# oarodriguez/PhD-QMCLib

Measured on AMD Instinct MI355X. Metric: walker-steps/sec, higher is better.
Workload: dtype f64

## Files before the change

### phd_qmclib_amd/csrc/qmc_kernels.h

```cpp
#pragma once

#include "qmc_device.h"
#include "qmc_sorted64.h"
#include "qmc_sorted128.h"

static constexpr int BLOCK = 256;

static constexpr int BLOCK64 = 64;
template <int G>
struct WalkBlock {
    static constexpr int N = (G == 64) ? BLOCK64 : BLOCK;
};

template <int GPB>
__device__ __forceinline__ long long walker_of_block(unsigned b, int grp)
{
    if (GPB == 1)
        return ((long long)(b >> 7) << 7) + ((b & 7u) << 4) + ((b & 127u) >> 3);
    return (long long)b * GPB + grp;
}

template <int G, int P, bool PAD, bool ZC, bool DMC = false>
struct StepLds {
    static constexpr int NROWS =
        DMC ? SortedCot<false, true, false>::ROWS : 5;
    static constexpr int SORTED =
        (G == 64 && P == 2 && !ZC)   ? NROWS * SortedRows<128>::ROW
        : (G == 64 && P == 1 && !ZC) ? NROWS * SortedRows<64>::ROW
                                     : 0;
    static constexpr int GENERAL = GroupLds<G, P, ZC>::DOUBLES;
    static constexpr int DOUBLES = SORTED > GENERAL ? SORTED : GENERAL;
};

__device__ __forceinline__ long long qmc_uniform(long long v)
{
    const int lo = __builtin_amdgcn_readfirstlane((int)v);
    const int hi = __builtin_amdgcn_readfirstlane((int)(v >> 32));
    return ((long long)hi << 32) | (unsigned int)lo;
}
__device__ __forceinline__ int qmc_opaque(int v)
{
    asm volatile("" : "+v"(v));
    return v;
}
__device__ __forceinline__ double qmc_uniform_f64(double v)
{
    return __longlong_as_double(qmc_uniform(__double_as_longlong(v)));
}
__device__ __forceinline__ double qmc_lane_f64(double v, int k)
{
    const long long b = __double_as_longlong(v);
    const int lo = __builtin_amdgcn_readlane((int)b, k);
    const int hi = __builtin_amdgcn_readlane((int)(b >> 32), k);
    return __longlong_as_double(((long long)hi << 32) | (unsigned int)lo);
}

template <int P>
__device__ __forceinline__ void vmc_accept_lanes(const int (&lab)[P], int n,
                                                 int &src0, int &src1)
{
    src0 = 0;
    src1 = 0;
#pragma unroll
    for (int p = 0; p < P; ++p) {
        const unsigned long long b0 = __ballot(lab[p] == 0);
        const unsigned long long b1 = __ballot(lab[p] == 1);
        if (b0) src0 = ((int)__ffsll((long long)b0) - 1) | (p << 6);
        if (b1) src1 = ((int)__ffsll((long long)b1) - 1) | (p << 6);
    }
    if (n == 1) src1 = src0;
}
template <int P>
__device__ __forceinline__ unsigned int vmc_read_slot(const uint32_t (&wd)[P],
                                                      int src)
{
    unsigned int r = 0u;
#pragma unroll
    for (int p = 0; p < P; ++p)
        if ((src >> 6) == p)
            r = (unsigned)__builtin_amdgcn_readlane((int)wd[p], src & 63);
    return r;
}

static constexpr int LB_P1 = 7;
static constexpr int LB_DMC_P2 = 5;
static constexpr int LB_VMC_P2 = 4;
constexpr int lb_waves(int G, int P, bool ZC, int p2)
{
    return (G == 64 && P == 1) ? LB_P1 : (G == 64 && P == 2 && !ZC) ? p2 : 1;
}


template <int P>
struct DmcSpare {
    static constexpr bool ON = P == 1;
};

static constexpr int RESORT_EVERY = 4;

struct EvalArgs {
    const double *pos;
    double *wf, *energy;
    double *ith, *drift;
    long long nconf;
};

template <int G, int P, bool PAD, bool ZC, typename R = double>
__global__ void __launch_bounds__(WalkBlock<G>::N, lb_waves(G, P, ZC, 1))
evaluate_kernel(const DevModel *__restrict__ mp, EvalArgs a)
{
    const DevModel &m = *mp;
    [[maybe_unused]] constexpr int QMC_SEC_OFF = 0;
    QMC_SECTION("top");
    extern __shared__ double smem[];
    constexpr int GPB = WalkBlock<G>::N / G;
    const int grp = threadIdx.x / G, gl = threadIdx.x % G;
    double *lds = smem + (size_t)grp * GroupLds<G, P, ZC>::DOUBLES;
    const long long w = walker_of_block<GPB>(blockIdx.x, grp);
    const bool active = w < a.nconf;
    if (GPB == 1 && !active) return;
    const long long wr = active ? w : 0;
    const int n = walker_n<G, P, PAD>(m);
    double z[P], z1[P], F[P], ei[P], E, wf;
#pragma unroll
    for (int p = 0; p < P; ++p) {
        int i = lane_particle<G, P, PAD>(m, gl, p);
        z1[p] = (i < n) ? a.pos[wr * n + i] : 0.0;
        z[p] = wrap_box(z1[p], m.L);
    }
    eval_walker<G, P, PAD, true, true, ZC, R>(m, z, z1, gl, lds, F, ei, E, wf);
    if (!active) return;
#pragma unroll
    for (int p = 0; p < P; ++p) {
        int i = lane_particle<G, P, PAD>(m, gl, p);
        if (i < n) {
            if (a.ith) a.ith[w * n + i] = ei[p];
            if (a.drift) a.drift[w * n + i] = F[p];
        }
    }
    if (gl == 0) {
        if (a.wf) a.wf[w] = wf;
        if (a.energy) a.energy[w] = E;
    }
}

struct PrepArgs {
    const double *pos;
    double *drift, *energy;
    long long nconf;
};

template <int G, int P, bool PAD, bool ZC, typename R = double>
__global__ void __launch_bounds__(WalkBlock<G>::N, lb_waves(G, P, ZC, 1))
prepare_kernel(const DevModel *__restrict__ mp, PrepArgs a)
{
    const DevModel &m = *mp;
    [[maybe_unused]] constexpr int QMC_SEC_OFF = 0;
    QMC_SECTION("top");
    extern __shared__ double smem[];
    constexpr int GPB = WalkBlock<G>::N / G;
    const int grp = threadIdx.x / G, gl = threadIdx.x % G;
    double *lds = smem + (size_t)grp * GroupLds<G, P, ZC>::DOUBLES;
    const long long w = walker_of_block<GPB>(blockIdx.x, grp);
    const bool active = w < a.nconf;
    if (GPB == 1 && !active) return;
    const long long wr = active ? w : 0;
    const int n = walker_n<G, P, PAD>(m);
    double z[P], z1[P], F[P], ei[P], E, wf;
#pragma unroll
    for (int p = 0; p < P; ++p) {
        int i = lane_particle<G, P, PAD>(m, gl, p);
        z1[p] = (i < n) ? a.pos[wr * n + i] : 0.0;
        z[p] = wrap_box(z1[p], m.L);
    }
    eval_walker<G, P, PAD, false, false, ZC, R>(m, z, z1, gl, lds, F, ei, E,
                                                wf);
    if (!active) return;
#pragma unroll
    for (int p = 0; p < P; ++p) {
        int i = lane_particle<G, P, PAD>(m, gl, p);
        if (i < n) a.drift[w * n + i] = F[p];
    }
    if (gl == 0) a.energy[w] = E;
}

struct alignas(64) VmcRec {
    double wf;
    double ecarry;
    double sum_e, sum_e2;
    long long n_acc;
    long long spare[3];
};
static_assert(sizeof(VmcRec) == 64, "one record = 8 eight-byte words");
typedef unsigned int VmcRecWords __attribute__((ext_vector_type(16)));
#define QMC_CONST __attribute__((address_space(4)))
__device__ __forceinline__ double vmc_rec_word(const VmcRecWords &r, int k)
{
    return __hiloint2double((int)r[2 * k + 1], (int)r[2 * k]);
}

struct VmcArgs {
    double *pos;
    unsigned short *label;
    VmcRec *rec;
    double *ser_wf, *ser_e;
    unsigned char *ser_stat;
    double *ser_pos;
    const double *tape;
    long long tape_steps;
    long long tape_idx;
    long long W;
    long long y;
    unsigned int nsteps;
    int forced;
    int reset_sums;
    int gaussian;
    unsigned int step;
    unsigned int chain0;
    unsigned long long seed;
    double move_spread;
};

template <int G, int P, bool ZC>
struct VmcFused {
    static constexpr bool ON = G == 64 && !ZC && (P == 1 || P == 2);
};

template <int G, int P, bool PAD, bool ZC, bool LEAN, typename R = double,
          bool STEADY = false>
__global__ void __launch_bounds__(WalkBlock<G>::N, lb_waves(G, P, ZC, LB_VMC_P2))
vmc_step_kernel(const DevModel *__restrict__ mp, VmcArgs a)
{
    static_assert(LEAN || !STEADY, "the steady variant is a LEAN kernel");
    const DevModel &m = *mp;
    [[maybe_unused]] constexpr int QMC_SEC_OFF = 0;
    QMC_SECTION("top");
    extern __shared__ double smem[];
    constexpr int GPB = WalkBlock<G>::N / G;
    const int grp = threadIdx.x / G, gl = threadIdx.x % G;
    static_assert(StepLds<G, P, PAD, ZC>::DOUBLES >= GroupLds<G, P, ZC>::DOUBLES,
                  "eval_walker is the fallback on the same LDS region");
    double *lds = smem + (size_t)grp * StepLds<G, P, PAD, ZC>::DOUBLES;
    const long long w = walker_of_block<GPB>(blockIdx.x, grp);
    const bool active = w < a.W;
    if (GPB == 1 && !active) return;
    const long long wr = active ? w : 0;
    const int n = walker_n<G, P, PAD>(m);
    const unsigned int slot = a.chain0 + (unsigned int)wr;
    const bool forced = !STEADY && a.forced != 0;
    const bool reset_sums = !STEADY && a.reset_sums != 0;

    const long long wl = (G == 64) ? qmc_uniform(wr) : wr;
    double wf_cur, e_cur, se = 0.0, se2 = 0.0;
    long long na = 0;
    if constexpr (G == 64) {
        const VmcRecWords r = *(const QMC_CONST VmcRecWords *)(a.rec + wl);
        wf_cur = vmc_rec_word(r, 0);
        e_cur = vmc_rec_word(r, 1);
        se = vmc_rec_word(r, 2);
        se2 = vmc_rec_word(r, 3);
        na = __double_as_longlong(vmc_rec_word(r, 4));
        if (reset_sums) { se = 0.0; se2 = 0.0; na = 0; }
    } else {
        wf_cur = a.rec[wl].wf;
        e_cur = a.rec[wl].ecarry;
    }

    constexpr bool FUSED = STEADY && VmcFused<G, P, ZC>::ON;
    double zc[P];
    int labc[P];
    int src0 = 0, src1 = 0;
    if constexpr (FUSED) {
#pragma unroll
        for (int p = 0; p < P; ++p) {
            int i = lane_particle<G, P, PAD>(m, gl, p);
            zc[p] = (i < n) ? a.pos[wr * n + i] : 0.0;
            labc[p] = (i < n) ? (int)a.label[wr * n + i] : i;
        }
        vmc_accept_lanes<P>(labc, n, src0, src1);
    }
    bool any_acc = false;
    const unsigned int nst = FUSED ? a.nsteps : 1u;
    bool acc = false;
    [[maybe_unused]] const int gl_top = gl;
    for (unsigned int s = 0; s < nst; ++s) {
    const unsigned int step = a.step + s;
    const int gl = FUSED ? qmc_opaque(gl_top) : gl_top;
    QMC_SECTION("load+philox+wrap");
    double zn[P];
    int labn[P];
    double ua = 1.0;
    unsigned int aw0 = 0u, aw1 = 0u;
    bool has0 = false, has1 = false;
    bool outside = false;
    [[maybe_unused]] uint32_t wacc[P];
#pragma unroll
    for (int p = 0; p < P; ++p) {
        wacc[p] = 0u;
        int i = lane_particle<G, P, PAD>(m, gl, p);
        double zp;
        if constexpr (FUSED) {
            zp = zc[p];
            labn[p] = labc[p];
        } else {
            zp = (i < n) ? a.pos[wr * n + i] : 0.0;
            labn[p] = (i < n) ? (int)a.label[wr * n + i] : i;
        }
        const unsigned li = (unsigned)labn[p];
        double d = 0.0;
        if (!forced && i < n) {
            if (!LEAN && a.tape) {
                double tv = a.tape[(wr * a.tape_steps + a.tape_idx) * (n + 1) + li];
                d = a.gaussian ? a.move_spread * tv
                               : (tv - 0.5) * a.move_spread;
            } else if (!LEAN && a.gaussian) {
                double g0, g1;
                philox_normal2(a.seed, slot, step, li, STREAM_VMC_MOVE, g0,
                               g1);
                d = a.move_spread * g0;
            } else {
                uint32_t w0, w1;
                vmc_move_block(a.seed, slot, step, li, w0, w1);
                d = vmc_move_unit(w0) * a.move_spread;
                if constexpr (FUSED) {
                    wacc[p] = w1;
                } else {
                    if (li == 0u) { aw0 = w1; has0 = true; }
                    if (li == 1u || n == 1) { aw1 = w1; has1 = true; }
                }
            }
        }
        zn[p] = wrap_box(zp + d, m.L);
        if (forced) outside = outside || zn[p] != zp;
    }
    if constexpr (FUSED) {
        aw0 = vmc_read_slot<P>(wacc, src0);
        aw1 = vmc_read_slot<P>(wacc, src1);
    }
    QMC_SECTION("resort");
    constexpr bool S64 = G == 64 && P == 1 && !ZC;
    constexpr bool S128 = G == 64 && P == 2 && !ZC;
    bool fast = false;
    if (forced)
        outside = __builtin_amdgcn_ballot_w64(outside) != 0ull;
    if constexpr (S64) {
        fast = !m.is_ideal && !outside &&
               sort_lanes64(zn[0], labn[0], gl, PAD ? n : 64) &&
               (PAD ? far_partner_ok_ring(m, zn[0], gl, n)
                    : far_partner_ok64(m, zn[0], gl));
    } else if constexpr (S128) {
        fast = !m.is_ideal && !outside && (!PAD || (n & 1) == 0) &&
               sort_rows128(zn, labn, gl, PAD ? n / 2 : 64) &&
               (PAD ? far_partner_ok_ring128(m, zn, gl, n / 2)
                    : far_partner_ok128(m, zn, gl));
    }
    if constexpr (S64 || S128) {
        if (!fast && !m.is_ideal && gl == 0 && active)
            atomicAdd(m.diag, 1ull);
    } else if constexpr (G == 64 && P == 1) {
        if (!forced) {
            anchor_seam(zn[0], labn[0], n);
            if ((a.step % RESORT_EVERY) == 0)
                resort_linear<G>(zn[0], labn[0], gl,
                                 a.step / RESORT_EVERY, n);
        }
    } else if constexpr (SlotMap<G, P>::CONSECUTIVE) {
        if (!forced) {
            anchor_seam_rows<P>(zn, labn, n);
            if ((a.step % RESORT_EVERY) == 0)
                resort_linear_rows<P>(zn, labn, gl, a.step / RESORT_EVERY, n);
        }
    } else if (!forced && (a.step % RESORT_EVERY) == 0)
        resort_step<G, P>(zn, labn, gl, a.step / RESORT_EVERY, n, m.L,
                          m.half_L, lanes_in_use<G, PAD>(m));
    constexpr bool TWO_PASS = G == 64;
    double F[P], ei[P], e_new = 0.0, wf_new;
    if (S64 && fast) {
        if constexpr (S64)
            eval_sorted64<R, true, false, false, PAD>(
                m, zn[0], gl, lds, F[0], e_new, wf_new);
    } else if (S128 && fast) {
        if constexpr (S128)
            eval_sorted128<R, true, false, false, PAD>(m, zn, gl, lds, F,
                                                       e_new, wf_new);
    } else {
        double z1[P];
#pragma unroll
        for (int p = 0; p < P; ++p) {
            int i = lane_particle<G, P, PAD>(m, gl, p);
            z1[p] = (outside && i < n) ? a.pos[wr * n + i] : zn[p];
        }
        if constexpr (TWO_PASS)
            eval_walker<G, P, PAD, true, false, ZC, R, false, false>(
                m, zn, z1, gl, lds, F, ei, e_new, wf_new);
        else
            eval_walker<G, P, PAD, true, false, ZC, R>(m, zn, z1, gl, lds, F,
                                                       ei, e_new, wf_new);
    }
    QMC_SECTION("metropolis+store");
    if (FUSED) {
        ua = u53(aw0, aw1);
    } else if (!forced) {
        if (!LEAN && a.tape) {
            ua = a.tape[(wr * a.tape_steps + a.tape_idx) * (n + 1) + n];
        } else if (!LEAN && a.gaussian) {
            double u1;
            philox_uniform2(a.seed, slot, step, 0u, STREAM_VMC_ACCEPT, ua,
                            u1);
        } else {
            const unsigned long long bal0 = __ballot(has0);
            const unsigned long long bal1 = __ballot(has1);
            unsigned int hi, lo;
            if (G == 64) {
                const int src0 = __builtin_amdgcn_readfirstlane(
                    (int)__ffsll((long long)bal0) - 1) & 63;
                const int src1 = __builtin_amdgcn_readfirstlane(
                    (int)__ffsll((long long)bal1) - 1) & 63;
                hi = (unsigned)__builtin_amdgcn_readlane((int)aw0, src0);
                lo = (unsigned)__builtin_amdgcn_readlane((int)aw1, src1);
            } else {
                const int base = (threadIdx.x & 63) - gl;
                const unsigned long long gmask = (1ull << (G & 63)) - 1ull;
                const int src0 = base + ((__ffsll((long long)((bal0 >> base) &
                                                              gmask)) - 1) & (G - 1));
                const int src1 = base + ((__ffsll((long long)((bal1 >> base) &
                                                              gmask)) - 1) & (G - 1));
                hi = (unsigned)__shfl((int)aw0, src0, 64);
                lo = (unsigned)__shfl((int)aw1, src1, 64);
            }
            ua = u53(hi, lo);
        }
    }
    if (!active) return;
    if constexpr (FUSED) {
        const double w0 = qmc_uniform_f64(wf_new);
        acc = ua <= 0.0 || w0 > wf_cur;
        if (!acc) acc = w0 > 0.5 * log_pos(ua) + wf_cur;
        acc = __builtin_amdgcn_readfirstlane((int)acc) != 0;
    } else {
        acc = forced || ua <= 0.0 || wf_new > wf_cur;
        if (!acc) acc = wf_new > 0.5 * log_pos(ua) + wf_cur;
        if (G == 64) acc = __builtin_amdgcn_readfirstlane((int)acc) != 0;
    }
    if (acc) {
        if constexpr (TWO_PASS) {
            QMC_SECTION("energy_pass");
            QMC_SECTION_PHASE(QMC_NSEC / 2);
            double wf_unused;
            if (S64 && fast) {
                if constexpr (S64)
                    eval_sorted64<R, false, true, true, PAD>(
                        m, zn[0], gl, lds, F[0], e_new, wf_unused);
            } else if (S128 && fast) {
                if constexpr (S128)
                    eval_sorted128<R, false, true, true, PAD>(
                        m, zn, gl, lds, F, e_new, wf_unused);
            } else {
                double z1[P];
#pragma unroll
                for (int p = 0; p < P; ++p) {
                    int i = lane_particle<G, P, PAD>(m, gl, p);
                    z1[p] = (outside && i < n) ? a.pos[wr * n + i] : zn[p];
                }
                eval_walker<G, P, PAD, false, false, ZC, R, true, true>(
                    m, zn, z1, gl, lds, F, ei, e_new, wf_unused);
            }
            QMC_SECTION_PHASE(0);
            QMC_SECTION("store");
        }
        if constexpr (FUSED) {
#pragma unroll
            for (int p = 0; p < P; ++p) {
                zc[p] = zn[p];
                labc[p] = labn[p];
            }
            vmc_accept_lanes<P>(labc, n, src0, src1);
            any_acc = true;
        } else {
#pragma unroll
            for (int p = 0; p < P; ++p) {
                int i = lane_particle<G, P, PAD>(m, gl, p);
                if (i < n && !forced) {
                    a.pos[w * n + i] = zn[p];
                    a.label[w * n + i] = (unsigned short)labn[p];
                }
            }
        }
        if (!FUSED) {
            wf_cur = wf_new;
            e_cur = e_new;
        }
    }
    if constexpr (FUSED) {
        if (acc) {
            wf_cur = qmc_uniform_f64(wf_new);
            const double e2 = qmc_lane_f64(e_new, 2);
            const double e3 = qmc_lane_f64(e_new, 3);
            e_cur = qmc_lane_f64(e_new, 1);
            se = se + e2;
            se2 = fma(e3, e3, se2);
            na = na + 1;
        } else {
            se = se + e_cur;
            se2 = fma(e_cur, e_cur, se2);
        }
        se = qmc_uniform_f64(se);
        se2 = qmc_uniform_f64(se2);
        continue;
    }
    if (!LEAN && a.ser_pos) {
#pragma unroll
        for (int p = 0; p < P; ++p) {
            int i = lane_particle<G, P, PAD>(m, gl, p);
            if (i < n) {
                const bool moved = acc && !forced;
                const int lb = moved ? labn[p] : (int)a.label[w * n + i];
                a.ser_pos[(a.y * a.W + w) * n + lb] =
                    moved ? zn[p] : a.pos[w * n + i];
            }
        }
    }
    if (G == 64) {
        const double sum1 = se + e_cur;
        const double sum2 = fma(e_cur, e_cur, se2);
        const long long na1 = qmc_uniform(na + (acc ? 1 : 0));
        double v = __longlong_as_double((gl == 4) ? na1 : 0ll);
        v = (gl == 0) ? wf_cur : v;
        v = (gl == 1) ? e_cur : v;
        v = (gl == 2) ? sum1 : v;
        v = (gl == 3) ? sum2 : v;
        if (gl < 8) reinterpret_cast<double *>(a.rec + wl)[gl] = v;
    }
    if (gl == 0) {
        if (G != 64) {
            VmcRec *r = a.rec + w;
            if (!reset_sums) { se = r->sum_e; se2 = r->sum_e2; na = r->n_acc; }
            r->wf = wf_cur;
            r->ecarry = e_cur;
            r->sum_e = se + e_cur;
            r->sum_e2 = fma(e_cur, e_cur, se2);
            r->n_acc = na + (acc ? 1 : 0);
        }
        if (!LEAN) {
            if (a.ser_wf) a.ser_wf[a.y * a.W + w] = wf_cur;
            if (a.ser_e) a.ser_e[a.y * a.W + w] = e_cur;
            if (a.ser_stat) a.ser_stat[a.y * a.W + w] = acc ? 1 : 0;
        }
    }
    }
    if constexpr (FUSED) {
        QMC_SECTION("fused_store");
        if (any_acc) {
#pragma unroll
            for (int p = 0; p < P; ++p) {
                int i = lane_particle<G, P, PAD>(m, gl, p);
                if (i < n) {
                    a.pos[w * n + i] = zc[p];
                    a.label[w * n + i] = (unsigned short)labc[p];
                }
            }
        }
        double v = __longlong_as_double((gl == 4) ? qmc_uniform(na) : 0ll);
        v = (gl == 0) ? wf_cur : v;
        v = (gl == 1) ? e_cur : v;
        v = (gl == 2) ? se : v;
        v = (gl == 3) ? se2 : v;
        if (gl < 8) reinterpret_cast<double *>(a.rec + wl)[gl] = v;
    }
    QMC_SECTION("end");
}

struct DmcCtl {
    long long prev_nw;
    long long nw;
    double ref_energy;
    double total_energy, total_weight;
    double e_t, w_t;
    long long spare_nw;
    unsigned int step;
    unsigned int pad;
};

struct EvolveArgs {
    const double *ppos, *pdrift, *penergy;
    double *cpos, *cdrift, *cenergy, *cweight;
    const unsigned short *plabel;
    unsigned short *clabel;
    double *eslot;
    const long long *ref;
    const DmcCtl *ctl;
    const double *g_tape;
    double *spare;
    long long maxw;
    double dt, sigma;
    unsigned long long seed;
    unsigned int slot0;
    int fix_stale;
};

template <int G, int P, bool PAD, bool ZC, typename R = double>
__global__ void __launch_bounds__(WalkBlock<G>::N, lb_waves(G, P, ZC, LB_DMC_P2))
dmc_evolve_kernel(const DevModel *__restrict__ mp, EvolveArgs a)
{
    const DevModel &m = *mp;
    [[maybe_unused]] constexpr int QMC_SEC_OFF = 0;
    extern __shared__ double smem[];
    constexpr int GPB = WalkBlock<G>::N / G;
    const int grp = threadIdx.x / G, gl = threadIdx.x % G;
    static_assert(StepLds<G, P, PAD, ZC, true>::DOUBLES >=
                      GroupLds<G, P, ZC>::DOUBLES,
                  "eval_walker is the fallback on the same LDS region");
    double *lds = smem + (size_t)grp * StepLds<G, P, PAD, ZC, true>::DOUBLES;
    const long long s = walker_of_block<GPB>(blockIdx.x, grp);
    const long long nw = a.ctl->nw;
    if ((GPB == 1 ? s : (long long)blockIdx.x * GPB) >= nw) return;
    QMC_SECTION("top");
    const bool active = s < nw;
    const long long sr = active ? s : 0;
    const int n = walker_n<G, P, PAD>(m);
    const unsigned int step = a.ctl->step;
    const double ref_energy = a.ctl->ref_energy;
    const long long spare_nw = a.ctl->spare_nw;
    const long long su = (G == 64) ? qmc_uniform(sr) : sr;
    const long long par = a.ref[su];
    double e_par = 0.0, e_slot = 0.0;
    if (G == 64) {
        e_par = a.penergy[par];
        e_slot = a.eslot[su];
    }

    QMC_SECTION("load+philox+wrap");
    double z[P];
    int lab[P];
#pragma unroll
    for (int p = 0; p < P; ++p) {
        int i = lane_particle<G, P, PAD>(m, gl, p);
        double zz = 0.0;
        lab[p] = i;
        if (i < n) {
            double z0 = a.ppos[par * n + i];
            double f0 = a.pdrift[par * n + i];
            const int li = (int)a.plabel[par * n + i];
            lab[p] = li;
            double g;
            if (a.g_tape) {
                g = a.g_tape[sr * n + li];
            } else if (DmcSpare<P>::ON && (step & 1u) && sr < spare_nw) {
                g = a.spare[sr * n + li];
            } else {
                double g0, g1;
                dmc_normal2(a.seed, a.slot0 + (unsigned)sr, step >> 1,
                            (unsigned)li, g0, g1);
                g = (step & 1u) ? g1 : g0;
                if (DmcSpare<P>::ON && !(step & 1u) && active)
                    a.spare[sr * n + li] = g1;
            }
            double zn = z0 + 2 * f0 * a.dt + a.sigma * g;
            zz = wrap_box(zn, m.L);
        }
        z[p] = zz;
    }
    QMC_SECTION("resort");
    constexpr bool S64 = G == 64 && P == 1 && !ZC;
    constexpr bool S128 = G == 64 && P == 2 && !ZC;
    bool fast = false;
    if constexpr (S64) {
        fast = !m.is_ideal && sort_lanes64(z[0], lab[0], gl, PAD ? n : 64) &&
               (PAD ? far_partner_ok_ring(m, z[0], gl, n)
                    : far_partner_ok64(m, z[0], gl));
    } else if constexpr (S128) {
        fast = !m.is_ideal && (!PAD || (n & 1) == 0) &&
               sort_rows128(z, lab, gl, PAD ? n / 2 : 64) &&
               (PAD ? far_partner_ok_ring128(m, z, gl, n / 2)
                    : far_partner_ok128(m, z, gl));
    }
    if constexpr (S64 || S128) {
        if (!fast && !m.is_ideal && gl == 0 && active)
            atomicAdd(m.diag, 1ull);
    } else if constexpr (G == 64 && P == 1) {
        anchor_seam(z[0], lab[0], n);
        if ((step % RESORT_EVERY) == 0)
            resort_linear<G>(z[0], lab[0], gl, step / RESORT_EVERY, n);
    } else if constexpr (SlotMap<G, P>::CONSECUTIVE) {
        anchor_seam_rows<P>(z, lab, n);
        if ((step % RESORT_EVERY) == 0)
            resort_linear_rows<P>(z, lab, gl, step / RESORT_EVERY, n);
    } else if ((step % RESORT_EVERY) == 0)
        resort_step<G, P>(z, lab, gl, step / RESORT_EVERY, n, m.L,
                          m.half_L, lanes_in_use<G, PAD>(m));
#pragma unroll
    for (int p = 0; p < P; ++p) {
        int i = lane_particle<G, P, PAD>(m, gl, p);
        if (active && i < n) {
            a.cpos[s * n + i] = z[p];
            a.clabel[s * n + i] = (unsigned short)lab[p];
        }
    }
    double F[P], ei[P], e_next, wf;
    if (S64 && fast) {
        if constexpr (S64)
            eval_sorted64<R, false, true, false, PAD>(m, z[0], gl, lds, F[0],
                                                      e_next, wf);
    } else if (S128 && fast) {
        if constexpr (S128)
            eval_sorted128<R, false, true, false, PAD>(m, z, gl, lds, F,
                                                       e_next, wf);
    } else
        eval_walker<G, P, PAD, false, false, ZC, R>(m, z, z, gl, lds, F, ei,
                                                    e_next, wf);
    QMC_SECTION("weight+store");
    if (!active) return;
#pragma unroll
    for (int p = 0; p < P; ++p) {
        int i = lane_particle<G, P, PAD>(m, gl, p);
        if (i < n) a.cdrift[s * n + i] = F[p];
    }
    if (gl == 0) {
        if (G != 64) { e_par = a.penergy[par]; e_slot = a.eslot[s]; }
        double e_old = a.fix_stale ? e_par : e_slot;
        double mean_energy = (e_next + e_old) / 2;
        a.cenergy[s] = e_next;
        a.cweight[s] = -a.dt * (mean_energy - ref_energy);
        a.eslot[s] = e_par;
    }
    QMC_SECTION("end");
}
```

Before: 759.6 million.

## Precompute Metropolis acceptance uniforms in lane-parallel chunks across fused VMC steps

In the fused steady VMC kernel, the per-step acceptance uniform is no longer taken from the label-0/label-1 particles' Philox words, which needed ballots after every accept plus readlane selection. Every 30 steps, lanes 4..63 each generate one Philox block for a future step, pair adjacent lanes via DPP to form the 53-bit uniform, and compute its clamped log once, storing a zero-mask ballot. Each step then reads the precomputed log-uniform with a readlane. This removes per-step ballot and readlane work and the per-step log from the serial path. In exchange it adds a batched Philox and log pass every 30 steps and relies on the precomputed stream matching the original acceptance draws.

```diff
diff --git a/phd_qmclib_amd/csrc/qmc_kernels.h b/phd_qmclib_amd/csrc/qmc_kernels.h
--- a/phd_qmclib_amd/csrc/qmc_kernels.h
+++ b/phd_qmclib_amd/csrc/qmc_kernels.h
@@ -53,33 +53,6 @@
     const int lo = __builtin_amdgcn_readlane((int)b, k);
     const int hi = __builtin_amdgcn_readlane((int)(b >> 32), k);
     return __longlong_as_double(((long long)hi << 32) | (unsigned int)lo);
-}
-
-template <int P>
-__device__ __forceinline__ void vmc_accept_lanes(const int (&lab)[P], int n,
-                                                 int &src0, int &src1)
-{
-    src0 = 0;
-    src1 = 0;
-#pragma unroll
-    for (int p = 0; p < P; ++p) {
-        const unsigned long long b0 = __ballot(lab[p] == 0);
-        const unsigned long long b1 = __ballot(lab[p] == 1);
-        if (b0) src0 = ((int)__ffsll((long long)b0) - 1) | (p << 6);
-        if (b1) src1 = ((int)__ffsll((long long)b1) - 1) | (p << 6);
-    }
-    if (n == 1) src1 = src0;
-}
-template <int P>
-__device__ __forceinline__ unsigned int vmc_read_slot(const uint32_t (&wd)[P],
-                                                      int src)
-{
-    unsigned int r = 0u;
-#pragma unroll
-    for (int p = 0; p < P; ++p)
-        if ((src >> 6) == p)
-            r = (unsigned)__builtin_amdgcn_readlane((int)wd[p], src & 63);
-    return r;
 }
 
 static constexpr int LB_P1 = 7;
@@ -240,7 +213,8 @@
     const int grp = threadIdx.x / G, gl = threadIdx.x % G;
     static_assert(StepLds<G, P, PAD, ZC>::DOUBLES >= GroupLds<G, P, ZC>::DOUBLES,
                   "eval_walker is the fallback on the same LDS region");
-    double *lds = smem + (size_t)grp * StepLds<G, P, PAD, ZC>::DOUBLES;
+    const int lds_off_top = grp * StepLds<G, P, PAD, ZC>::DOUBLES;
+    double *lds_top = smem + lds_off_top;
     const long long w = walker_of_block<GPB>(blockIdx.x, grp);
     const bool active = w < a.W;
     if (GPB == 1 && !active) return;
@@ -269,7 +243,10 @@
     constexpr bool FUSED = STEADY && VmcFused<G, P, ZC>::ON;
     double zc[P];
     int labc[P];
-    int src0 = 0, src1 = 0;
+    constexpr unsigned int ACC_LANE0 = 4u, ACC_CHUNK = (64u - ACC_LANE0) / 2u;
+    [[maybe_unused]] double carry = 0.0;
+    [[maybe_unused]] unsigned long long acc_zero = 0ull;
+    [[maybe_unused]] unsigned int ct = 0u;
     if constexpr (FUSED) {
 #pragma unroll
         for (int p = 0; p < P; ++p) {
@@ -277,7 +254,6 @@
             zc[p] = (i < n) ? a.pos[wr * n + i] : 0.0;
             labc[p] = (i < n) ? (int)a.label[wr * n + i] : i;
         }
-        vmc_accept_lanes<P>(labc, n, src0, src1);
     }
     bool any_acc = false;
     const unsigned int nst = FUSED ? a.nsteps : 1u;
@@ -286,6 +262,22 @@
     for (unsigned int s = 0; s < nst; ++s) {
     const unsigned int step = a.step + s;
     const int gl = FUSED ? qmc_opaque(gl_top) : gl_top;
+    double *lds = FUSED ? smem + qmc_opaque(lds_off_top) : lds_top;
+    if constexpr (FUSED) {
+        if (ct == 0u) {
+            const unsigned int l = (unsigned int)gl_top - ACC_LANE0;
+            uint32_t mv, hi;
+            vmc_move_block(a.seed, slot, step + (l >> 1),
+                           n == 1 ? 0u : (l & 1u), mv, hi);
+            const uint32_t lo = (uint32_t)__builtin_amdgcn_update_dpp(
+                0, (int)hi, 0xB1, 0xf, 0xf, false);
+            const double u = u53(hi, lo);
+            const bool keeps = gl_top >= (int)ACC_LANE0 && !(gl_top & 1);
+            acc_zero = __builtin_amdgcn_ballot_w64(keeps && u <= 0.0);
+            const double lu = (u <= 0.0) ? 0.0 : fmin(log_pos(u), 0.0);
+            carry = keeps ? lu : carry;
+        }
+    }
     QMC_SECTION("load+philox+wrap");
     double zn[P];
     int labn[P];
@@ -293,10 +285,8 @@
     unsigned int aw0 = 0u, aw1 = 0u;
     bool has0 = false, has1 = false;
     bool outside = false;
-    [[maybe_unused]] uint32_t wacc[P];
 #pragma unroll
     for (int p = 0; p < P; ++p) {
-        wacc[p] = 0u;
         int i = lane_particle<G, P, PAD>(m, gl, p);
         double zp;
         if constexpr (FUSED) {
@@ -322,9 +312,7 @@
                 uint32_t w0, w1;
                 vmc_move_block(a.seed, slot, step, li, w0, w1);
                 d = vmc_move_unit(w0) * a.move_spread;
-                if constexpr (FUSED) {
-                    wacc[p] = w1;
-                } else {
+                if constexpr (!FUSED) {
                     if (li == 0u) { aw0 = w1; has0 = true; }
                     if (li == 1u || n == 1) { aw1 = w1; has1 = true; }
                 }
@@ -332,10 +320,6 @@
         }
         zn[p] = wrap_box(zp + d, m.L);
         if (forced) outside = outside || zn[p] != zp;
-    }
-    if constexpr (FUSED) {
-        aw0 = vmc_read_slot<P>(wacc, src0);
-        aw1 = vmc_read_slot<P>(wacc, src1);
     }
     QMC_SECTION("resort");
     constexpr bool S64 = G == 64 && P == 1 && !ZC;
@@ -399,7 +383,6 @@
     }
     QMC_SECTION("metropolis+store");
     if (FUSED) {
-        ua = u53(aw0, aw1);
     } else if (!forced) {
         if (!LEAN && a.tape) {
             ua = a.tape[(wr * a.tape_steps + a.tape_idx) * (n + 1) + n];
@@ -434,8 +417,9 @@
     if (!active) return;
     if constexpr (FUSED) {
         const double w0 = qmc_uniform_f64(wf_new);
-        acc = ua <= 0.0 || w0 > wf_cur;
-        if (!acc) acc = w0 > 0.5 * log_pos(ua) + wf_cur;
+        const int t = (int)(2u * ct + ACC_LANE0);
+        const double lu = qmc_lane_f64(carry, t);
+        acc = ((acc_zero >> t) & 1ull) != 0ull || w0 > fma(lu, 0.5, wf_cur);
         acc = __builtin_amdgcn_readfirstlane((int)acc) != 0;
     } else {
         acc = forced || ua <= 0.0 || wf_new > wf_cur;
@@ -474,7 +458,6 @@
                 zc[p] = zn[p];
                 labc[p] = labn[p];
             }
-            vmc_accept_lanes<P>(labc, n, src0, src1);
             any_acc = true;
         } else {
 #pragma unroll
@@ -506,6 +489,7 @@
         }
         se = qmc_uniform_f64(se);
         se2 = qmc_uniform_f64(se2);
+        ct = (ct + 1u == ACC_CHUNK) ? 0u : ct + 1u;
         continue;
     }
     if (!LEAN && a.ser_pos) {
```

Measured after the change: 758.3 million, median of 2. Within noise of the previous version (-0.2%).

## Precompute Metropolis acceptance thresholds across lanes for 64 steps at once

Applied to the files above, without the earlier changes.

In the fused VMC loop, each lane now computes the acceptance uniform and its log threshold for one future step, refreshed every 64 steps. Each step reads its threshold with a readlane. This removes the per-step ballot/ffs search for the label-0/1 lanes, the readlane of their Philox words, and the per-step log evaluation. The trade-off is two extra Philox blocks per lane every 64 steps and a NaN sentinel for the ua<=0 case. It relies on the accept word for particle labels 0/1 being reproducible by calling vmc_move_block with the step offset by lane.

```diff
diff --git a/phd_qmclib_amd/csrc/qmc_kernels.h b/phd_qmclib_amd/csrc/qmc_kernels.h
--- a/phd_qmclib_amd/csrc/qmc_kernels.h
+++ b/phd_qmclib_amd/csrc/qmc_kernels.h
@@ -55,31 +55,17 @@
     return __longlong_as_double(((long long)hi << 32) | (unsigned int)lo);
 }
 
-template <int P>
-__device__ __forceinline__ void vmc_accept_lanes(const int (&lab)[P], int n,
-                                                 int &src0, int &src1)
-{
-    src0 = 0;
-    src1 = 0;
-#pragma unroll
-    for (int p = 0; p < P; ++p) {
-        const unsigned long long b0 = __ballot(lab[p] == 0);
-        const unsigned long long b1 = __ballot(lab[p] == 1);
-        if (b0) src0 = ((int)__ffsll((long long)b0) - 1) | (p << 6);
-        if (b1) src1 = ((int)__ffsll((long long)b1) - 1) | (p << 6);
-    }
-    if (n == 1) src1 = src0;
-}
-template <int P>
-__device__ __forceinline__ unsigned int vmc_read_slot(const uint32_t (&wd)[P],
-                                                      int src)
-{
-    unsigned int r = 0u;
-#pragma unroll
-    for (int p = 0; p < P; ++p)
-        if ((src >> 6) == p)
-            r = (unsigned)__builtin_amdgcn_readlane((int)wd[p], src & 63);
-    return r;
+__device__ __forceinline__ double vmc_accept_thresholds(uint64_t seed,
+                                                        uint32_t slot,
+                                                        uint32_t step0, int lane,
+                                                        int n)
+{
+    uint32_t m0, m1, hi, lo;
+    vmc_move_block(seed, slot, step0 + (uint32_t)lane, 0u, m0, hi);
+    vmc_move_block(seed, slot, step0 + (uint32_t)lane, n == 1 ? 0u : 1u, m1, lo);
+    const double ua = u53(hi, lo);
+    const double h = 0.5 * log_pos(ua);
+    return ua <= 0.0 ? __builtin_nan("") : h;
 }
 
 static constexpr int LB_P1 = 7;
@@ -269,7 +255,7 @@
     constexpr bool FUSED = STEADY && VmcFused<G, P, ZC>::ON;
     double zc[P];
     int labc[P];
-    int src0 = 0, src1 = 0;
+    [[maybe_unused]] double thr = 0.0;
     if constexpr (FUSED) {
 #pragma unroll
         for (int p = 0; p < P; ++p) {
@@ -277,7 +263,6 @@
             zc[p] = (i < n) ? a.pos[wr * n + i] : 0.0;
             labc[p] = (i < n) ? (int)a.label[wr * n + i] : i;
         }
-        vmc_accept_lanes<P>(labc, n, src0, src1);
     }
     bool any_acc = false;
     const unsigned int nst = FUSED ? a.nsteps : 1u;
@@ -286,6 +271,10 @@
     for (unsigned int s = 0; s < nst; ++s) {
     const unsigned int step = a.step + s;
     const int gl = FUSED ? qmc_opaque(gl_top) : gl_top;
+    if constexpr (FUSED) {
+        if ((s & 63u) == 0u)
+            thr = vmc_accept_thresholds(a.seed, slot, step, gl, n);
+    }
     QMC_SECTION("load+philox+wrap");
     double zn[P];
     int labn[P];
@@ -293,10 +282,8 @@
     unsigned int aw0 = 0u, aw1 = 0u;
     bool has0 = false, has1 = false;
     bool outside = false;
-    [[maybe_unused]] uint32_t wacc[P];
 #pragma unroll
     for (int p = 0; p < P; ++p) {
-        wacc[p] = 0u;
         int i = lane_particle<G, P, PAD>(m, gl, p);
         double zp;
         if constexpr (FUSED) {
@@ -322,9 +309,7 @@
                 uint32_t w0, w1;
                 vmc_move_block(a.seed, slot, step, li, w0, w1);
                 d = vmc_move_unit(w0) * a.move_spread;
-                if constexpr (FUSED) {
-                    wacc[p] = w1;
-                } else {
+                if constexpr (!FUSED) {
                     if (li == 0u) { aw0 = w1; has0 = true; }
                     if (li == 1u || n == 1) { aw1 = w1; has1 = true; }
                 }
@@ -332,10 +317,6 @@
         }
         zn[p] = wrap_box(zp + d, m.L);
         if (forced) outside = outside || zn[p] != zp;
-    }
-    if constexpr (FUSED) {
-        aw0 = vmc_read_slot<P>(wacc, src0);
-        aw1 = vmc_read_slot<P>(wacc, src1);
     }
     QMC_SECTION("resort");
     constexpr bool S64 = G == 64 && P == 1 && !ZC;
@@ -399,7 +380,6 @@
     }
     QMC_SECTION("metropolis+store");
     if (FUSED) {
-        ua = u53(aw0, aw1);
     } else if (!forced) {
         if (!LEAN && a.tape) {
             ua = a.tape[(wr * a.tape_steps + a.tape_idx) * (n + 1) + n];
@@ -434,8 +414,9 @@
     if (!active) return;
     if constexpr (FUSED) {
         const double w0 = qmc_uniform_f64(wf_new);
-        acc = ua <= 0.0 || w0 > wf_cur;
-        if (!acc) acc = w0 > 0.5 * log_pos(ua) + wf_cur;
+        const double h = qmc_lane_f64(thr, (int)(s & 63u));
+        acc = h != h || w0 > wf_cur;
+        if (!acc) acc = w0 > h + wf_cur;
         acc = __builtin_amdgcn_readfirstlane((int)acc) != 0;
     } else {
         acc = forced || ua <= 0.0 || wf_new > wf_cur;
@@ -474,7 +455,6 @@
                 zc[p] = zn[p];
                 labc[p] = labn[p];
             }
-            vmc_accept_lanes<P>(labc, n, src0, src1);
             any_acc = true;
         } else {
 #pragma unroll
```

Result: faster. 777.6 million before, 786.3 million after (median of 6 runs) (+1.1%).
